# Deam0on/deepEMIA

Hardware: AMD Instinct MI355X
Metric: EM tiles/s (2048x2048, R101-FPN) (higher is better)
Workload: dtype f16x2

## Files before the change

deepemia_amd/_lib.py:

```python
from __future__ import annotations

import ctypes as C
import os
from pathlib import Path

_HERE = Path(__file__).resolve().parent
LIB_PATH = _HERE / "csrc" / ("libdeepemia_hip_dev.so" if os.environ.get("DEEPEMIA_DEV_LIB", "0") == "1" else "libdeepemia_hip.so")

F32, BF16, F32X3, BF16X2, F16X2, P32 = 0, 1, 2, 3, 4, 5
ACT_NONE, ACT_RELU, ACT_SIGMOID = 0, 1, 2
RES_NONE, RES_SAME, RES_UP2 = 0, 1, 2
MOP = {"fill": 1, "dilate": 2, "erode": 3, "drop_multi": 4, "flag_multi": 5, "gate": 6}


class HipExtensionMissing(RuntimeError):
    pass


class HipKernelError(RuntimeError):
    pass


class ConvDesc(C.Structure):
    _fields_ = [
# ... 8 lines not shown
    ]


class ConvP32Desc(C.Structure):
    _fields_ = [
        ("in_", C.c_void_p), ("in_meta", C.c_void_p), ("w", C.c_void_p), ("scale", C.c_void_p), ("bias", C.c_void_p),
        ("residual", C.c_void_p), ("res_meta", C.c_void_p), ("out", C.c_void_p), ("out_meta", C.c_void_p),
        ("wbound", C.c_float), ("bbound", C.c_float),
        ("N", C.c_int32), ("H", C.c_int32), ("W", C.c_int32), ("Cin", C.c_int32),
        ("Ho", C.c_int32), ("Wo", C.c_int32), ("Cout", C.c_int32), ("CoutPad", C.c_int32),
        ("KH", C.c_int32), ("KW", C.c_int32), ("stride", C.c_int32), ("pad", C.c_int32),
        ("act", C.c_int32), ("res_mode", C.c_int32), ("out_f32", C.c_int32), ("out_ld", C.c_int32), ("tile_hint", C.c_int32),
        ("head_w", C.c_void_p), ("head_b", C.c_void_p), ("head_out", C.c_void_p),
        ("head_n", C.c_int32), ("head_ld", C.c_int32), ("head_act", C.c_int32),
        ("groups", C.c_int32), ("group_rows", C.c_int32), ("row0", C.c_int32), ("single", C.c_int32),
    ]


class RpnDesc(C.Structure):
    _fields_ = [
        ("head", C.c_void_p * 5), ("H", C.c_int32 * 5), ("W", C.c_int32 * 5), ("stride", C.c_int32 * 5),
        ("cell_anchors", C.c_void_p), ("head_ld", C.c_int32), ("N", C.c_int32),
        ("img_h", C.c_int32), ("img_w", C.c_int32), ("pre_topk", C.c_int32), ("post_topk", C.c_int32),
        ("nms_thresh", C.c_float), ("out_boxes", C.c_void_p), ("out_scores", C.c_void_p),
        ("out_count", C.c_void_p), ("workspace", C.c_void_p),
    ]


class RoiAlignDesc(C.Structure):
    _fields_ = [
# ... 212 lines not shown
```

deepemia_amd/csrc/conv_p32.hip:

```cpp
#include <utility>
#include "common.h"
#ifndef P32_ABLATE
#define P32_ABLATE 0
#endif

#ifndef P32_HEAD_DIRECT
#define P32_HEAD_DIRECT 1
#endif
#ifndef P32_SINGLE
#define P32_SINGLE 0
#endif
#ifndef P32_DEV_TILES
#define P32_DEV_TILES 0
#endif
#ifndef P32_ST_AUX
#define P32_ST_AUX 0
#endif
#ifndef P32_RES_AUX
#define P32_RES_AUX 0
#endif
#ifndef P32_A_NT
#define P32_A_NT 0
#endif
#ifndef P32_FRAG_PIPE
// ... 11 lines not shown
    const void* res;
    const float* res_meta;
    void* out;
    float* out_meta;
    float wbound, bbound;
    int N, H, W, Cin, Ho, Wo, Cout, CoutPad, KH, KW, stride, pad;
    int act, res_mode, out_f32, out_ld;
    int M, HoWo, ntn, nwg, ksteps, taps;
    int kloop;
    unsigned in_bytes, w_bytes;
    unsigned out_bytes, res_bytes;
    const float* head_w;
    const float* head_b;
    float* head_out;
    int head_n, head_ld, head_act;
    int groups, group_rows, row0;
    int no_hk;
    int zero_low;
    int stagger_ticks;
    int resident;
};

typedef __attribute__((address_space(3))) void lds_void;

template <int OFF, int WAIT>
__device__ __forceinline__ void ds_read2_b128(f16x8& a, f16x8& b, unsigned addr_a, unsigned addr_b) {
    if constexpr (WAIT >= 0)
        asm volatile("ds_read_b128 %0, %2 offset:%4\n\tds_read_b128 %1, %3 offset:%4\n\ts_waitcnt lgkmcnt(%5)"
                     : "=&v"(a), "=&v"(b) : "v"(addr_a), "v"(addr_b), "n"(OFF), "n"(WAIT) : "memory");
    else
// ... 73 lines not shown
    if (p.res_mode != DEMIA_RES_NONE) { amax_res = p.res_meta[2 * gi]; s_res = p.res_meta[2 * gi + 1]; }
    post = uniform(1.0f / s_in);
    resi = uniform(p.res_mode != DEMIA_RES_NONE ? 1.0f / s_res : 0.f);
    sout = uniform(planes_out ? plane_scale(amax_in * p.wbound + p.bbound + amax_res) : 1.f);
}

__device__ __forceinline__ GroupScales load_group_scales(const ConvQ& p, int m0, bool planes_out) {
    GroupScales gs;
    gs.g0 = (m0 + p.row0) / p.group_rows;
    gs.b1 = (gs.g0 + 1) * p.group_rows - p.row0;
    gs.b2 = gs.b1 + p.group_rows;
    load_group_scale(p, gs.g0, planes_out, gs.post0, gs.resi0, gs.sout0);
    load_group_scale(p, gs.g0 + 1, planes_out, gs.post1, gs.resi1, gs.sout1);
    load_group_scale(p, gs.g0 + 2, planes_out, gs.post2, gs.resi2, gs.sout2);
    return gs;
}

template <int WM, int WN, int TM, int TN, bool HEAD, typename WriteRow>
__device__ __forceinline__ void p32_epilogue(const ConvQ& p, const GroupScales& gs, char* smem, WriteRow&& write_tile_row, int wm, int wn, int m0, int n0) {
    constexpr int BN = WN * TN * 32;
    const int tid = threadIdx.x, lane = tid & 63;
    constexpr int EROW = BN * 4 + 16;
    constexpr int GPR = BN / 8, RSTEP = 512 / GPR, ITEMS = WM * 32 / RSTEP;
    static_assert(512 % GPR == 0 && (WM * 32) % RSTEP == 0, "epilogue split");
    constexpr int BM_ = WM * TM * 32;
    static_assert(!HEAD || BN == 256, "the fused head needs a 256-wide tile");
    const bool planes_out = !HEAD && !p.out_f32;
    const int g0 = __builtin_amdgcn_readfirstlane(gs.g0), b1 = __builtin_amdgcn_readfirstlane(gs.b1), b2 = __builtin_amdgcn_readfirstlane(gs.b2);
    const float post0 = uniform(gs.post0), post1 = uniform(gs.post1), post2 = uniform(gs.post2);
    const float resi0 = uniform(gs.resi0), resi1 = uniform(gs.resi1), resi2 = uniform(gs.resi2);
// ... 64 lines not shown
#pragma unroll
        for (int k = 0; k < ITEMS; ++k) { ch[k] = rh[k]; cl[k] = rl[k]; }
        if (i + 1 < TM) load_res(i + 1);
        if (co < p.Cout) {
#pragma unroll
            for (int k = 0; k < ITEMS; ++k) {
                const int lr = r_first + k * RSTEP;
                const int m = row_of(i, k);
                if (m >= p.M) continue;
                const float4 x0 = *reinterpret_cast<const float4*>(smem + lr * EROW + g * 32);
                const float4 x1 = *reinterpret_cast<const float4*>(smem + lr * EROW + g * 32 + 16);
                float v[8] = {x0.x, x0.y, x0.z, x0.w, x1.x, x1.y, x1.z, x1.w};
                const int gd = (m >= b1) + (m >= b2);
                const float post = gd == 0 ? post0 : (gd == 1 ? post1 : post2);
#pragma unroll
                for (int q = 0; q < 8; ++q) v[q] = (v[q] * post) * sc[q] + bs[q];
                if (res_on) {
                    const float res_inv = gd == 0 ? resi0 : (gd == 1 ? resi1 : resi2);
#pragma unroll
                    for (int q = 0; q < 8; ++q) v[q] += ((float)ch[k][q] + (float)cl[k][q]) * res_inv;
                }
#pragma unroll
                for (int q = 0; q < 8; ++q) v[q] = fmaxf(v[q], act_lo);
                if (sigmoid_on) {
#pragma unroll
                    for (int q = 0; q < 8; ++q) v[q] = 1.0f / (1.0f + expf(-v[q]));
                }
                if (head_on) {
                    float acc_h[HMAX];
#pragma unroll
                    for (int j = 0; j < HMAX; ++j) {
// ... 145 lines not shown
        asm volatile("" ::: "memory");
        __builtin_amdgcn_wave_barrier();
        f16x8 ch[ITEMS], cl[ITEMS];
#pragma unroll
        for (int k = 0; k < ITEMS; ++k) {
            ch[k] = __builtin_bit_cast(f16x8, from_below(rh[k], rl[k]));
            cl[k] = __builtin_bit_cast(f16x8, from_above(rl[k], rh[k]));
        }
        if (i + 1 < TM) load_res(i + 1);
#pragma unroll
        for (int k = 0; k < ITEMS; ++k) {
            const int lr = r_first + k * RPI;
            const int m = row_of(i, k);
            const float4 x0 = *reinterpret_cast<const float4*>(wsm + lr * (LDW * 4) + (line * 4 + cj) * 32);
            const float4 x1 = *reinterpret_cast<const float4*>(wsm + lr * (LDW * 4) + (line * 4 + cj) * 32 + 16);
            typedef float f32x2 __attribute__((ext_vector_type(2)));
            f32x2 v2[4] = {{x0.x, x0.y}, {x0.z, x0.w}, {x1.x, x1.y}, {x1.z, x1.w}};
            const int gd = (m >= b1) + (m >= b2);
            const float post = gd == 0 ? post0 : (gd == 1 ? post1 : post2);
            const float res_inv = gd == 0 ? resi0 : (gd == 1 ? resi1 : resi2);
            const float s_out = gd == 0 ? sout0 : (gd == 1 ? sout1 : sout2);
            float v[8];
#pragma unroll
            for (int q = 0; q < 4; ++q) {
                const f32x2 scq = {sc[2 * q], sc[2 * q + 1]}, bsq = {bs[2 * q], bs[2 * q + 1]};
                const f32x2 t = (v2[q] * post) * scq + bsq;
                v[2 * q] = t.x;
                v[2 * q + 1] = t.y;
            }
#pragma unroll
            for (int q = 0; q < 8; ++q) {
                v[q] = fmaf((float)cl[k][q], res_inv, fmaf((float)ch[k][q], res_inv, v[q]));
                v[q] = fmaxf(v[q], act_lo);
            }
            if (sigmoid_on && !(P32_ABLATE & 256)) {
#pragma unroll
                for (int q = 0; q < 8; ++q) v[q] = 1.0f / (1.0f + expf(-v[q]));
            }
            f16x8 h, l;
            float vm = 0.f;
#pragma unroll
            for (int q = 0; q < 8; q += 2) {
                vm = fmaxf(vm, fmaxf(fabsf(v[q]), fabsf(v[q + 1])));
                const f32x2 y = f32x2{v[q], v[q + 1]} * s_out;
                h[q] = (_Float16)y.x;
                h[q + 1] = (_Float16)y.y;
                l[q] = (_Float16)fmaf(-(float)h[q], 1.0f, y.x);
                l[q + 1] = (_Float16)fmaf(-(float)h[q + 1], 1.0f, y.y);
            }
            if (single) l = f16x8{0, 0, 0, 0, 0, 0, 0, 0};
            vm = m < p.M ? vm : 0.f;
            vmax0 = fmaxf(vmax0, gd == 0 ? vm : 0.f);
            vmax1 = fmaxf(vmax1, gd == 1 ? vm : 0.f);
            vmax2 = fmaxf(vmax2, gd == 2 ? vm : 0.f);
            const u32x4 hu = __builtin_bit_cast(u32x4, h), lu = __builtin_bit_cast(u32x4, l);
            const u32x4 d0 = from_below(hu, lu);
            const u32x4 d1 = from_above(lu, hu);
            const unsigned off = (unsigned)(m - rs) * cbytes + lofs;
            if (P32_ABLATE & 64) {
                asm volatile("" :: "v"(d0), "v"(d1), "v"(off));
            } else {
                __builtin_amdgcn_raw_buffer_store_b128(d0, rs_out, off, 0, P32_ST_AUX);
                __builtin_amdgcn_raw_buffer_store_b128(d1, rs_out, off + cbytes, 0, P32_ST_AUX);
            }
// ... 66 lines not shown
    const int tile_n_ = n0 / BN;
    for (int o = tid; o < BM * HN; o += WM * WN * 64) {
        const int row = o / HN, j = o - row * HN;
        const int m = m0 + row;
        if (m >= p.M || j >= p.head_n) continue;
        float z = 0.f;
#pragma unroll
        for (int w = 0; w < WN; ++w) z += part[((long)w * BM + row) * HN + j];
        z += p.head_b[j];
        p.head_out[((long)m * p.ntn + tile_n_) * p.head_ld + j] =
            p.head_act == DEMIA_ACT_SIGMOID ? 1.0f / (1.0f + expf(-z)) : (p.head_act == DEMIA_ACT_RELU ? fmaxf(z, 0.f) : z);
    }
}


constexpr int EPI_GENERIC = 0, EPI_PLANES = 1, EPI_HEAD = 2;

template <int WM, int WN, int TM, int TN, bool M16 = true, int EPI = EPI_PLANES, int NST = 2, bool HK = false>
__global__ __launch_bounds__(WM * WN * 64, WM * WN == 8 ? 2 : 1) void conv_p32_kernel(const ConvQ p) {
    static_assert(NST == 2 || NST == 3, "two or three LDS stages");
    static_assert(!HK || (P32_SINGLE && M16 && NST == 2), "HK is a variant of the single-plane 16x16x32 kernel");
    static_assert(WM * WN == 8 || (WM * WN == 4 && EPI == EPI_PLANES), "eight waves, or four (planes epilogue only)");
    constexpr int NW = WM * WN;
    constexpr int BM = WM * TM * 32, BN = WN * TN * 32;
    constexpr int STAGE = (BM + BN) * 128;
    constexpr int NIA = BM / 8, NIB = BN / 8;

    extern __shared__ __attribute__((aligned(16))) char smem[];
    const int tid = threadIdx.x, lane = tid & 63;
    const int wave = __builtin_amdgcn_readfirstlane(tid >> 6);
    const int wm = wave / WN, wn = wave % WN;
// ... 324 lines not shown
            asm volatile("s_waitcnt lgkmcnt(0)\n\ts_barrier" ::: "memory");
        } else if (!BARRIER_IN_COMPUTE) {
            asm volatile("s_waitcnt vmcnt(0) lgkmcnt(0)\n\ts_barrier" ::: "memory");
        }
        st = NST == 2 ? (st ^ 1) : (st == 2 ? 0 : st + 1);
    }
#undef P32_ADVANCE

    if constexpr ((P32_ABLATE & 2048) != 0 && M16) {
#pragma unroll
        for (int i = 0; i < 2 * TM; ++i)
#pragma unroll
            for (int j = 0; j < 2 * TN; ++j) asm volatile("" :: "v"(acc16[i][j]));
        return;
    }
    if constexpr (EPI == EPI_PLANES) {
        if constexpr (M16) {
            p32_epilogue_planes<WM, WN, TM, TN>(p, gs, smem, [&](int i, float* e) { write_acc16<TN, TN * 32 + 4>(acc16[2 * i], acc16[2 * i + 1], e, lane); }, wm, wn, m0, n0);
        } else {
            p32_epilogue_planes<WM, WN, TM, TN>(p, gs, smem, [&](int i, float* e) { write_acc32<TN, TN * 32 + 4>(acc[i], e, lane); }, wm, wn, m0, n0);
        }
    } else if constexpr (M16 && HEAD && P32_HEAD_DIRECT) {
        if (p.act != DEMIA_ACT_SIGMOID && p.head_n <= 2)
            p32_epilogue_head_direct<WM, WN, TM, TN, 2>(p, gs, smem, acc16, wm, wn, m0, n0);
        else
            p32_epilogue<WM, WN, TM, TN, HEAD>(p, gs, smem, [&](int i, float* e) { write_acc16<TN, BN + 4>(acc16[2 * i], acc16[2 * i + 1], e, lane); }, wm, wn, m0, n0);
    } else if constexpr (M16) {
        p32_epilogue<WM, WN, TM, TN, HEAD>(p, gs, smem, [&](int i, float* e) { write_acc16<TN, BN + 4>(acc16[2 * i], acc16[2 * i + 1], e, lane); }, wm, wn, m0, n0);
    } else {
        p32_epilogue<WM, WN, TM, TN, HEAD>(p, gs, smem, [&](int i, float* e) { write_acc32<TN, BN + 4>(acc[i], e, lane); }, wm, wn, m0, n0);
    }
}

#if P32_DEV_TILES
#include "conv_p32_dev.inc"
#endif

template <int WM, int WN, int TM, int TN, bool M16 = true, int EPI = EPI_PLANES, int NST = 2, bool HK = false>
int launch_q_(ConvQ p, hipStream_t st) {
    constexpr int BM = WM * TM * 32, BN = WN * TN * 32;
    constexpr int stages = NST * (BM + BN) * 128, image = EPI == EPI_PLANES ? WM * WN * 32 * (TN * 128 + 16) : WM * 32 * (BN * 4 + 16);
    static_assert(stages <= 160 * 1024, "LDS");
    constexpr int smem = stages > image ? stages : image;
    p.ntn = p.CoutPad / BN;
    p.nwg = p.ntn * cdiv(p.M, BM);
    p.resident = 256 * (160 * 1024 / smem >= 2 ? 2 : 1);
    p.kloop = HK ? p.ksteps / 2 : p.ksteps;
    auto k = conv_p32_kernel<WM, WN, TM, TN, M16, EPI, NST, HK>;
    static bool attr_done = false;
    if (!attr_done) {
        (void)hipFuncSetAttribute(reinterpret_cast<const void*>(k), hipFuncAttributeMaxDynamicSharedMemorySize, smem);
        attr_done = true;
    }
    hipLaunchKernelGGL(k, dim3(p.nwg), dim3(WM * WN * 64), smem, st, p);
    DEMIA_CHECK_LAUNCH("conv_p32_kernel");
    return DEMIA_OK;
}
// ... 32 lines not shown
        const double t = predict_us(c, M, cout_pad, ksteps, residual);
        if (t < best_t) { best_t = t; best = c.id; }
    }
    return best;
}

}

#if P32_SINGLE
extern "C" int demia_conv2d_p32_single(const demia_conv_p32_desc* d, void* stream) {
#else
extern "C" int demia_conv2d_p32_single(const demia_conv_p32_desc* d, void* stream);
extern "C" int demia_conv2d_p32(const demia_conv_p32_desc* d, void* stream) {
    if (d && d->single) return demia_conv2d_p32_single(d, stream);
#endif
    DEMIA_REQUIRE(d && d->in && d->in_meta && d->w && (d->out || d->head_n > 0), "null pointer");
    DEMIA_REQUIRE(d->out_f32 || d->out_meta || d->head_n > 0, "P32 output needs out_meta");
    DEMIA_REQUIRE(d->Cin > 0 && d->Cin % 32 == 0, "Cin must be a multiple of 32");
    DEMIA_REQUIRE(d->CoutPad >= d->Cout && d->CoutPad % 64 == 0, "CoutPad must be a multiple of 64");
    DEMIA_REQUIRE(d->out_f32 || d->Cout % 32 == 0, "P32 output needs Cout % 32 == 0");
    DEMIA_REQUIRE(d->KH > 0 && d->KW > 0 && d->KH * d->KW <= 32 && d->stride > 0 && d->pad >= 0, "kernel geometry");
    DEMIA_REQUIRE(d->Ho == (d->H + 2 * d->pad - d->KH) / d->stride + 1, "Ho");
    DEMIA_REQUIRE(d->Wo == (d->W + 2 * d->pad - d->KW) / d->stride + 1, "Wo");
    DEMIA_REQUIRE(d->res_mode == DEMIA_RES_NONE || (d->residual && d->res_meta), "residual pointer");
    DEMIA_REQUIRE((long)d->N * d->Ho * d->Wo < (1L << 31), "M overflow");
    const long in_bytes = 128 + (long)d->N * d->H * d->W * d->Cin * 4;
    DEMIA_REQUIRE(in_bytes < (1L << 32), "input planes must stay below 4 GiB");
    const long w_bytes = (long)d->CoutPad * d->KH * d->KW * d->Cin * 4;
    DEMIA_REQUIRE(w_bytes < (1L << 31), "weight planes must stay below 2 GiB");
    ConvQ p;
    p.in = d->in; p.in_meta = d->in_meta; p.w = d->w; p.scale = d->scale; p.bias = d->bias;
    p.res = d->residual; p.res_meta = d->res_meta; p.out = d->out; p.out_meta = d->out_meta;
// ... 14 lines not shown
        static const char* env = getenv("DEMIA_P32_NO_HK");
        p.no_hk = (env && env[0] == '1') ? 1 : 0;
    }
    p.kloop = 0;
    p.resident = 256;
    p.groups = d->groups > 1 ? d->groups : 1;
    p.group_rows = p.groups > 1 ? d->group_rows : (1 << 29);
    p.row0 = p.groups > 1 ? d->row0 : 0;
    DEMIA_REQUIRE(p.groups == 1 || (d->group_rows >= 128 && d->row0 >= 0 && ((long)p.M + d->row0 + d->group_rows - 1) / d->group_rows <= p.groups),
                  "scale groups: group_rows >= 128 and the rows of this call must fall inside `groups` groups");
    p.head_w = d->head_w; p.head_b = d->head_b; p.head_out = d->head_out; p.head_n = d->head_n; p.head_ld = d->head_ld; p.head_act = d->head_act;
    if (d->head_n > 0) {
        DEMIA_REQUIRE(d->head_n <= 4 && d->head_w && d->head_b && d->head_out && d->head_ld >= d->head_n, "fused head: at most 4 rows, pointers, head_ld");
        DEMIA_REQUIRE(d->CoutPad % 256 == 0 && d->Cout == d->CoutPad && !d->out_f32, "fused head needs Cout % 256 == 0 and a planes layer");
    }
    p.stagger_ticks = 0;
#if P32_DEV_TILES
    {
        static const char* env = getenv("DEMIA_P32_STAGGER_US");
        p.stagger_ticks = env ? atoi(env) * 100 : 0;
    }
#endif
    if (p.M == 0) return DEMIA_OK;
    hipStream_t st = reinterpret_cast<hipStream_t>(stream);
    int tile = d->tile_hint ? d->tile_hint : choose_tile(p.M, d->CoutPad, p.ksteps, d->res_mode != DEMIA_RES_NONE, d->head_n > 0);
    const bool n256 = d->CoutPad % 256 == 0, n128 = d->CoutPad % 128 == 0;
    if (d->head_n > 0) {
        switch (tile) {
            case 1: return launch_q<2, 4, 4, 2, true, EPI_HEAD>(p, st);
            case 2: return launch_q<2, 4, 2, 2, true, EPI_HEAD>(p, st);
            default: return launch_q<1, 8, 6, 1, true, EPI_HEAD>(p, st);
        }
    }
    const int tile_bn = (tile == 9 || tile == 10 || tile == 11 || tile == 49) ? 64 : ((tile >= 6 && tile <= 8) || tile == 26 ? 128 : 256);
    const long out_bytes = 128 + (long)p.M * d->Cout * 4;
    long res_bytes = 0;
    if (d->res_mode == DEMIA_RES_SAME) res_bytes = out_bytes;
    if (d->res_mode == DEMIA_RES_UP2) res_bytes = 128 + (long)d->N * ((d->Ho + 1) / 2) * ((d->Wo + 1) / 2) * d->Cout * 4;
    const bool planes = !d->out_f32 && d->Cout % tile_bn == 0 && out_bytes < (1L << 32) - 512 && res_bytes < (1L << 32) - 512 &&
                        (long)(p.M + 256) * d->Cout * 4 + 256 < (1L << 32);
    p.out_bytes = (unsigned)out_bytes; p.res_bytes = (unsigned)res_bytes;
// ... 49 lines not shown
```

deepemia_amd/engine.py:

```python
from __future__ import annotations

import os

import ctypes as C
import math
from dataclasses import dataclass
from typing import Dict, List, Optional, Sequence, Tuple

import numpy as np
import torch

from . import _lib, p32
from ._lib import ACT_NONE, ACT_RELU, ACT_SIGMOID, BF16, BF16X2, F16X2, F32, F32X3, RES_NONE, RES_SAME, RES_UP2

RES_BLOCKS = {50: (3, 4, 6, 3), 101: (3, 4, 23, 3)}
PIXEL_MEAN = (103.530, 116.280, 123.675)
ANCHOR_SIZES = (32, 64, 128, 256, 512)
ANCHOR_RATIOS = (0.5, 1.0, 2.0)
STRIDES = (4, 8, 16, 32, 64)
DEFAULT_SINGLE_STAGES = ()
MASK_HEAD_STAGES = ("mask_fcn", "deconv")
STAGES = ("res2", "res3", "res4", "res5", "fpn_lateral", "fpn_output", "rpn_conv", "rpn_pred", "fc1", "fc2", "box_pred", "mask_fcn", "deconv")
BN_EPS = 1e-5
PRE_NMS_TOPK = 1000
# ... 213 lines not shown
        self._graphs: Dict[tuple, dict] = {}
        self._arena: Dict[tuple, list] = {}
        self._arena_key: Optional[tuple] = None
        self._arena_i = 0
        self._paste_static = None
        self.stem_mode = os.environ.get("DEEPEMIA_STEM", "fused") if self.p32 else "valu"
        self.stem_on_mfma = self.stem_mode in ("fused", "mfma")
        self.max_cached_shapes = max(1, int(os.environ.get("DEEPEMIA_MAX_CACHED_SHAPES", "3")))
        self._shape_lru: List[tuple] = []
        self.evictions = 0
        self.dt = BF16 if precision == "bf16" else F32
        self.tdt = torch.bfloat16 if precision == "bf16" else torch.float32
        self._tables: Dict[Tuple[int, int], dict] = {}
        self._cell = cell_anchor_table()
        self.roi_order = os.environ.get("DEEPEMIA_ROI_ORDER", "0") == "1"
        self.conv_events = None
        self.unmatched_keys: List[str] = []
        self._used = set()
        self._pack(state_dict)

    def _get(self, sd, key):
        if key not in sd:
            raise KeyError(f"checkpoint is missing '{key}' (expected Detectron2 0.6 Mask R-CNN R{self.depth}-FPN layout)")
        self._used.add(key)
        return sd[key].detach().to(torch.float32).cpu()

    def _conv(self, sd, prefix, stride=1, pad=0, norm=False, bias=False, weight=None, bias_t=None, stage: str = "") -> ConvLayer:
        w = self._get(sd, prefix + ".weight") if weight is None else weight
        cout, cin, kh, kw = w.shape
        cout_pad = (cout + 63) // 64 * 64 if self.p32 else (cout + 31) // 32 * 32
# ... 171 lines not shown
        m = self._meta_pool[self._meta_i]
        self._meta_i += 1
        return m

    def new_p32(self, shape, groups: Optional[int] = None) -> p32.P32:
        n = 1
        for d in shape:
            n *= int(d)
        buf = self._scratch(p32.HEADER_HALFS + 2 * n, torch.float16, zero_head=p32.HEADER_HALFS)
        return p32.P32(buf, self._meta_slot(self._groups if groups is None else groups), tuple(int(d) for d in shape))

    def dense(self, x) -> torch.Tensor:
        return p32.to_f32(x) if isinstance(x, p32.P32) else x.float()

    def conv_p32(self, x: p32.P32, L: ConvLayer, act=ACT_NONE, residual: Optional[p32.P32] = None, res_mode=RES_NONE,
                 out_f32: bool = False, out_ld: int = 0, tile_hint: int = 0, head=None):
        n, h, w, cin = x.shape
        assert cin == L.cin, (cin, L.cin)
        ho = (h + 2 * L.pad - L.kh) // L.stride + 1
        wo = (w + 2 * L.pad - L.kw) // L.stride + 1
        hw_ptr = hb_ptr = ho_ptr = hn = hld = hact = 0
        if head is not None:
            hw_t, hb_t, hld, hact = head
            hn = int(hw_t.shape[0])
            out = self._scratch(n * ho * wo * (L.cout // 256) * hld, torch.float32).view(n * ho * wo * (L.cout // 256), hld)
            hw_ptr, hb_ptr, ho_ptr = _lib.ptr(hw_t), _lib.ptr(hb_t), _lib.ptr(out)
            optr, ometa = 0, 0
        elif out_f32:
            ld = out_ld if out_ld > 0 else L.cout
            out = self._scratch(n * ho * wo * ld, torch.float32).view(n, ho, wo, ld)
            optr, ometa = _lib.ptr(out), 0
        else:
            out = self.new_p32((n, ho, wo, L.cout), x.groups)
            optr, ometa = _lib.ptr(out.buf), _lib.ptr(out.meta)
        pix_bytes = cin * 4
        limit = (1 << 32) - (1 << 20)
        chunks = [(0, n)]
# ... 4 lines not shown
            chunks = [(i, min(step, n - i)) for i in range(0, n, step)]
        ev = self.conv_events
        if ev is not None:
            e0, e1 = torch.cuda.Event(enable_timing=True), torch.cuda.Event(enable_timing=True)
            e0.record(torch.cuda.current_stream(self.device))
        groups = x.groups
        group_rows = (n * ho * wo) // groups
        assert groups == 1 or (group_rows * groups == n * ho * wo and (residual is None or residual.groups == groups)), (x.shape, groups)
        for c0, cn in chunks:
            d = _lib.ConvP32Desc(_lib.ptr(x.buf) + c0 * pix_bytes, _lib.ptr(x.meta), _lib.ptr(L.w3), _lib.ptr(L.scale3), _lib.ptr(L.bias),
                                 0 if residual is None else _lib.ptr(residual.buf) + c0 * L.cout * 4,
                                 0 if residual is None else _lib.ptr(residual.meta),
                                 (optr + c0 * (ld if out_f32 else L.cout) * 4) if optr else 0, ometa, L.wbound, L.bbound, cn, h, w, cin,
                                 ho, wo, L.cout, L.cout_pad, L.kh, L.kw, L.stride, L.pad, act, res_mode, 1 if out_f32 else 0, out_ld,
                                 tile_hint, hw_ptr, hb_ptr, (ho_ptr + c0 * (L.cout // 256) * hld * 4) if ho_ptr else 0, hn, hld, hact,
                                 groups, group_rows, c0, L.single)
            _lib.check(self.lib.demia_conv2d_p32(C.byref(d), self._stream()), "demia_conv2d_p32")
        if ev is not None:
            e1.record(torch.cuda.current_stream(self.device))
            nbytes = (n * h * w * cin * 4 + L.cout_pad * L.kh * L.kw * cin * 4 + n * ho * wo * L.cout * 4 +
                      (0 if residual is None else residual.pixels * residual.channels * 4))
            ev.append((e0, e1, 2.0 * n * ho * wo * L.cout * L.kh * L.kw * cin, "f16" if L.single else self.precision, nbytes))
        return out

    def conv(self, x, L: ConvLayer, act=ACT_NONE, residual=None, res_mode=RES_NONE,
             out_dtype=None, out: Optional[torch.Tensor] = None, out_ld: int = 0, tile_hint: int = 0):
        if self.p32:
            return self.conv_p32(x, L, act, residual, res_mode, out_f32=out_dtype is not None, out_ld=out_ld, tile_hint=tile_hint)
        n, h, w, cin = x.shape
        assert cin == L.cin, (cin, L.cin)
        ho = (h + 2 * L.pad - L.kh) // L.stride + 1
        wo = (w + 2 * L.pad - L.kw) // L.stride + 1
        odt = self.tdt if out_dtype is None else out_dtype
        ld = out_ld if out_ld > 0 else L.cout
        if out is None:
            out = torch.empty((n, ho, wo, ld), dtype=odt, device=self.device)
        use3 = L.w3 is not None and odt == torch.float32
# ... 144 lines not shown
        h5, w5 = p5.shape[1], p5.shape[2]
        if self.p32:
            p6 = self.new_p32((b, (h5 - 1) // 2 + 1, (w5 - 1) // 2 + 1, 256))
            p6 = p32.P32(p6.buf, p5.meta, p6.shape)
            _lib.check(self.lib.demia_subsample2(_lib.ptr(p5.buf) + 128, _lib.ptr(p6.buf) + 128, b, h5, w5, 256, F32, st), "demia_subsample2")
            feats["p6"] = p6
            return feats
        p6 = torch.empty((b, (h5 - 1) // 2 + 1, (w5 - 1) // 2 + 1, 256), dtype=self.tdt, device=self.device)
        _lib.check(self.lib.demia_subsample2(_lib.ptr(p5), _lib.ptr(p6), b, h5, w5, 256, self.dt, st), "demia_subsample2")
        feats["p6"] = p6
        return feats

    def rpn(self, feats, newh: int, neww: int):
        b = feats["p2"].shape[0]
        heads = []
        for name in ("p2", "p3", "p4", "p5", "p6"):
            t = self.conv(feats[name], self.rpn_conv, act=ACT_RELU)
            heads.append(self.conv(t, self.rpn_pred, out_dtype=torch.float32, out_ld=16))
        boxes = torch.empty((b, POST_NMS_TOPK, 4), dtype=torch.float32, device=self.device)
        scores = torch.empty((b, POST_NMS_TOPK), dtype=torch.float32, device=self.device)
        count = torch.empty((b,), dtype=torch.int32, device=self.device)
        ws = torch.empty((int(self.lib.demia_rpn_workspace_bytes(b)),), dtype=torch.uint8, device=self.device)
        d = _lib.RpnDesc()
        for i, hd in enumerate(heads):
            d.head[i] = _lib.ptr(hd)
            d.H[i], d.W[i], d.stride[i] = hd.shape[1], hd.shape[2], STRIDES[i]
        d.cell_anchors = self._cell.ctypes.data
        d.head_ld, d.N, d.img_h, d.img_w = 16, b, newh, neww
        d.pre_topk, d.post_topk, d.nms_thresh = PRE_NMS_TOPK, POST_NMS_TOPK, RPN_NMS_THRESH
        d.out_boxes, d.out_scores, d.out_count, d.workspace = _lib.ptr(boxes), _lib.ptr(scores), _lib.ptr(count), _lib.ptr(ws)
        _lib.check(self.lib.demia_rpn_proposals(C.byref(d), self._stream()), "demia_rpn_proposals")
# ... 175 lines not shown
```

include/deepemia_hip.h:

```cpp
#ifndef DEEPEMIA_HIP_H
#define DEEPEMIA_HIP_H

#include <stdint.h>

#ifdef __cplusplus
extern "C" {
#endif

#define DEMIA_OK 0
#define DEMIA_EINVAL (-1)
#define DEMIA_ELAUNCH (-2)

#define DEMIA_F32 0
#define DEMIA_BF16 1
#define DEMIA_F32X3 2
#define DEMIA_BF16X2 3
#define DEMIA_F16X2 4
#define DEMIA_P32 5

#define DEMIA_ACT_NONE 0
#define DEMIA_ACT_RELU 1
#define DEMIA_ACT_SIGMOID 2

#define DEMIA_RES_NONE 0
// ... 41 lines not shown
    float* out_meta;
    float wbound, bbound;
    int32_t N, H, W, Cin;
    int32_t Ho, Wo, Cout, CoutPad;
    int32_t KH, KW, stride, pad;
    int32_t act, res_mode;
    int32_t out_f32;
    int32_t out_ld;
    int32_t tile_hint;
    const float* head_w;
    const float* head_b;
    float* head_out;
    int32_t head_n, head_ld, head_act;
    int32_t groups, group_rows, row0;
    int32_t single;
} demia_conv_p32_desc;
int demia_conv2d_p32(const demia_conv_p32_desc* d, void* stream);

int demia_resize_h_u8(const uint8_t* src, uint8_t* tmp, int N, int H, int W, int newW,
                      const int32_t* xmin, const int32_t* xsize, const int32_t* xk, int ksx, void* stream);
int demia_resize_v_norm(const uint8_t* tmp, void* dst, int N, int H, int newW, int newH, int PH, int PW,
                        const int32_t* ymin, const int32_t* ysize, const int32_t* yk, int ksy,
                        const float* mean3, int dtype, void* stream);

int demia_resize_linear_u8(const uint8_t* src, uint8_t* dst, int N, int H, int W, int out_h, int out_w,
                           const int32_t* xofs, const int16_t* ialpha, const int32_t* yofs, const int16_t* ibeta,
                           void* stream);

int demia_stem_conv(const void* in, const void* w, const float* scale, const float* bias, void* mid,
                    int N, int PH, int PW, int dtype, void* stream);
// ... 222 lines not shown
```

Measured before the change: 719.5.

## Fuse RPN 1x1 prediction conv into the 3x3 RPN conv epilogue

Adds an epilogue mode to the P32 conv kernel that, for the 256-channel RPN 3x3 conv, writes the activated tile as f16 hi/lo planes into LDS and immediately runs the following 1x1 prediction layer (up to 16 outputs) with MFMA, storing f32 head outputs directly. The goal is to avoid materialising the 256-channel intermediate in HBM and to save a second kernel launch per FPN level. The fused path is on by default for f16x2 and adds LDS pressure, an extra barrier per row tile, and a new tile choice. The shared elementwise code is factored into a helper.

```diff
diff --git a/deepemia_amd/_lib.py b/deepemia_amd/_lib.py
--- a/deepemia_amd/_lib.py
+++ b/deepemia_amd/_lib.py
@@ -46,6 +46,7 @@
         ("head_w", C.c_void_p), ("head_b", C.c_void_p), ("head_out", C.c_void_p),
         ("head_n", C.c_int32), ("head_ld", C.c_int32), ("head_act", C.c_int32),
         ("groups", C.c_int32), ("group_rows", C.c_int32), ("row0", C.c_int32), ("single", C.c_int32),
+        ("head_planes", C.c_void_p), ("head_scale", C.c_void_p), ("head_bias", C.c_void_p), ("head_cout", C.c_int32),
     ]
 
 
diff --git a/deepemia_amd/csrc/conv_p32.hip b/deepemia_amd/csrc/conv_p32.hip
--- a/deepemia_amd/csrc/conv_p32.hip
+++ b/deepemia_amd/csrc/conv_p32.hip
@@ -49,6 +49,10 @@
     const float* head_b;
     float* head_out;
     int head_n, head_ld, head_act;
+    const void* hp_w;
+    const float* hp_scale;
+    const float* hp_bias;
+    int hp_cout;
     int groups, group_rows, row0;
     int no_hk;
     int zero_low;
@@ -152,6 +156,41 @@
     load_group_scale(p, gs.g0 + 1, planes_out, gs.post1, gs.resi1, gs.sout1);
     load_group_scale(p, gs.g0 + 2, planes_out, gs.post2, gs.resi2, gs.sout2);
     return gs;
+}
+
+__device__ __forceinline__ float scale_shift(float acc, float post, float sc, float bs) { return (acc * post) * sc + bs; }
+__device__ __forceinline__ void planes_item(const float4 x0, const float4 x1, float post, float res_inv, float s_out, const float (&sc)[8],
+                                            const float (&bs)[8], const f16x8 ch, const f16x8 cl, float act_lo, bool sigmoid_on,
+                                            f16x8& h, f16x8& l, float& vm) {
+    typedef float f32x2 __attribute__((ext_vector_type(2)));
+    f32x2 v2[4] = {{x0.x, x0.y}, {x0.z, x0.w}, {x1.x, x1.y}, {x1.z, x1.w}};
+    float v[8];
+#pragma unroll
+    for (int q = 0; q < 4; ++q) {
+        const f32x2 scq = {sc[2 * q], sc[2 * q + 1]}, bsq = {bs[2 * q], bs[2 * q + 1]};
+        const f32x2 t = (v2[q] * post) * scq + bsq;
+        v[2 * q] = t.x;
+        v[2 * q + 1] = t.y;
+    }
+#pragma unroll
+    for (int q = 0; q < 8; ++q) {
+        v[q] = fmaf((float)cl[q], res_inv, fmaf((float)ch[q], res_inv, v[q]));
+        v[q] = fmaxf(v[q], act_lo);
+    }
+    if (sigmoid_on && !(P32_ABLATE & 256)) {
+#pragma unroll
+        for (int q = 0; q < 8; ++q) v[q] = 1.0f / (1.0f + expf(-v[q]));
+    }
+    vm = 0.f;
+#pragma unroll
+    for (int q = 0; q < 8; q += 2) {
+        vm = fmaxf(vm, fmaxf(fabsf(v[q]), fabsf(v[q + 1])));
+        const f32x2 y = f32x2{v[q], v[q + 1]} * s_out;
+        h[q] = (_Float16)y.x;
+        h[q + 1] = (_Float16)y.y;
+        l[q] = (_Float16)fmaf(-(float)h[q], 1.0f, y.x);
+        l[q + 1] = (_Float16)fmaf(-(float)h[q + 1], 1.0f, y.y);
+    }
 }
 
 template <int WM, int WN, int TM, int TN, bool HEAD, typename WriteRow>
@@ -246,7 +285,7 @@
                 const int gd = (m >= b1) + (m >= b2);
                 const float post = gd == 0 ? post0 : (gd == 1 ? post1 : post2);
 #pragma unroll
-                for (int q = 0; q < 8; ++q) v[q] = (v[q] * post) * sc[q] + bs[q];
+                for (int q = 0; q < 8; ++q) v[q] = scale_shift(v[q], post, sc[q], bs[q]);
                 if (res_on) {
                     const float res_inv = gd == 0 ? resi0 : (gd == 1 ? resi1 : resi2);
 #pragma unroll
@@ -422,40 +461,13 @@
             const int m = row_of(i, k);
             const float4 x0 = *reinterpret_cast<const float4*>(wsm + lr * (LDW * 4) + (line * 4 + cj) * 32);
             const float4 x1 = *reinterpret_cast<const float4*>(wsm + lr * (LDW * 4) + (line * 4 + cj) * 32 + 16);
-            typedef float f32x2 __attribute__((ext_vector_type(2)));
-            f32x2 v2[4] = {{x0.x, x0.y}, {x0.z, x0.w}, {x1.x, x1.y}, {x1.z, x1.w}};
             const int gd = (m >= b1) + (m >= b2);
             const float post = gd == 0 ? post0 : (gd == 1 ? post1 : post2);
             const float res_inv = gd == 0 ? resi0 : (gd == 1 ? resi1 : resi2);
             const float s_out = gd == 0 ? sout0 : (gd == 1 ? sout1 : sout2);
-            float v[8];
-#pragma unroll
-            for (int q = 0; q < 4; ++q) {
-                const f32x2 scq = {sc[2 * q], sc[2 * q + 1]}, bsq = {bs[2 * q], bs[2 * q + 1]};
-                const f32x2 t = (v2[q] * post) * scq + bsq;
-                v[2 * q] = t.x;
-                v[2 * q + 1] = t.y;
-            }
-#pragma unroll
-            for (int q = 0; q < 8; ++q) {
-                v[q] = fmaf((float)cl[k][q], res_inv, fmaf((float)ch[k][q], res_inv, v[q]));
-                v[q] = fmaxf(v[q], act_lo);
-            }
-            if (sigmoid_on && !(P32_ABLATE & 256)) {
-#pragma unroll
-                for (int q = 0; q < 8; ++q) v[q] = 1.0f / (1.0f + expf(-v[q]));
-            }
             f16x8 h, l;
-            float vm = 0.f;
-#pragma unroll
-            for (int q = 0; q < 8; q += 2) {
-                vm = fmaxf(vm, fmaxf(fabsf(v[q]), fabsf(v[q + 1])));
-                const f32x2 y = f32x2{v[q], v[q + 1]} * s_out;
-                h[q] = (_Float16)y.x;
-                h[q + 1] = (_Float16)y.y;
-                l[q] = (_Float16)fmaf(-(float)h[q], 1.0f, y.x);
-                l[q + 1] = (_Float16)fmaf(-(float)h[q + 1], 1.0f, y.y);
-            }
+            float vm;
+            planes_item(x0, x1, post, res_inv, s_out, sc, bs, ch[k], cl[k], act_lo, sigmoid_on, h, l, vm);
             if (single) l = f16x8{0, 0, 0, 0, 0, 0, 0, 0};
             vm = m < p.M ? vm : 0.f;
             vmax0 = fmaxf(vmax0, gd == 0 ? vm : 0.f);
@@ -552,7 +564,115 @@
 }
 
 
-constexpr int EPI_GENERIC = 0, EPI_PLANES = 1, EPI_HEAD = 2;
+template <int WM, int WN, int TM, int TN>
+struct HeadPlanesLds {
+    static constexpr int LDW = TN * 32 + 4, ROWS = WM * 32;
+    static constexpr int STG = WM * WN * 32 * LDW * 4, IMG = ROWS * 8 * 128, WB = 8 * 16 * 128;
+    static constexpr int BYTES = STG + IMG + WB;
+};
+template <int WM, int WN, int TM, int TN, typename WriteRow>
+__device__ __forceinline__ void p32_epilogue_head_planes(const ConvQ& p, const GroupScales& gs, char* smem, WriteRow&& write_tile_row, int wm, int wn, int m0) {
+    typedef HeadPlanesLds<WM, WN, TM, TN> L;
+    static_assert(WN * TN == 8 && WM * WN == 8, "one N tile of 256 channels, eight waves");
+    constexpr int LDW = L::LDW, ROWS = L::ROWS;
+    constexpr int PPW = 8 / TN, RPI = 2 * PPW, ITEMS = 32 / RPI;
+    const int tid = threadIdx.x, lane = tid & 63;
+    const int wave = __builtin_amdgcn_readfirstlane(tid >> 6);
+    char* const wsm = smem + wave * (32 * LDW * 4);
+    char* const img = smem + L::STG;
+    char* const wimg = img + L::IMG;
+    const int b1 = __builtin_amdgcn_readfirstlane(gs.b1), b2 = __builtin_amdgcn_readfirstlane(gs.b2);
+    const float post0 = uniform(gs.post0), post1 = uniform(gs.post1), post2 = uniform(gs.post2);
+    const float sout0 = uniform(gs.sout0), sout1 = uniform(gs.sout1), sout2 = uniform(gs.sout2);
+    const float ipost0 = uniform(1.0f / sout0), ipost1 = uniform(1.0f / sout1), ipost2 = uniform(1.0f / sout2);
+    u32x4 wreg[2];
+#pragma unroll
+    for (int q = 0; q < 2; ++q) {
+        const int c = tid + q * 512, g = c >> 7, row = (c >> 3) & 15, ck = c & 7;
+        wreg[q] = *reinterpret_cast<const u32x4*>(reinterpret_cast<const char*>(p.hp_w) + g * 8192 + row * 128 + ck * 16);
+    }
+    const int cj = lane & 3, rs = (lane >> 2) & 1, lg = lane >> 3;
+    const int line = lg % TN;
+    const int r_first = (lg / TN) * 2 + rs;
+    const int cgrp = wn * TN + line;
+    const int co = (cgrp * 4 + cj) * 8;
+    float sc[8], bs[8];
+#pragma unroll
+    for (int q = 0; q < 8; ++q) {
+        sc[q] = p.scale ? p.scale[co + q] : 1.0f;
+        bs[q] = p.bias ? p.bias[co + q] : 0.0f;
+    }
+    const bool sigmoid_on = p.act == DEMIA_ACT_SIGMOID;
+    const float act_lo = p.act == DEMIA_ACT_RELU ? 0.f : -INFINITY;
+    const f16x8 zero8 = {0, 0, 0, 0, 0, 0, 0, 0};
+    const int r16 = lane & 15, kq = lane >> 4, fsw = (r16 >> 1) & 7;
+    const bool c_ok = r16 < p.hp_cout;
+    const float hsc = (p.hp_scale && c_ok) ? p.hp_scale[r16] : 1.0f;
+    const float hbs = (p.hp_bias && c_ok) ? p.hp_bias[r16] : 0.0f;
+#pragma unroll
+    for (int i = 0; i < TM; ++i) {
+        asm volatile("" ::: "memory");
+        __builtin_amdgcn_wave_barrier();
+        write_tile_row(i, reinterpret_cast<float*>(wsm));
+        asm volatile("" ::: "memory");
+        __builtin_amdgcn_wave_barrier();
+        f16x8 h[ITEMS], l[ITEMS];
+#pragma unroll
+        for (int k = 0; k < ITEMS; ++k) {
+            const int lr = r_first + k * RPI;
+            const int m = m0 + wm * (TM * 32) + i * 32 + lr;
+            const float4 x0 = *reinterpret_cast<const float4*>(wsm + lr * (LDW * 4) + (line * 4 + cj) * 32);
+            const float4 x1 = *reinterpret_cast<const float4*>(wsm + lr * (LDW * 4) + (line * 4 + cj) * 32 + 16);
+            const int gd = (m >= b1) + (m >= b2);
+            const float post = gd == 0 ? post0 : (gd == 1 ? post1 : post2);
+            const float s_out = gd == 0 ? sout0 : (gd == 1 ? sout1 : sout2);
+            float vm;
+            planes_item(x0, x1, post, 0.f, s_out, sc, bs, zero8, zero8, act_lo, sigmoid_on, h[k], l[k], vm);
+        }
+        if (i > 0) __syncthreads();
+#pragma unroll
+        for (int k = 0; k < ITEMS; ++k) {
+            const int R = wm * 32 + r_first + k * RPI, sw = (R >> 1) & 7;
+            char* ln = img + (cgrp * ROWS + R) * 128;
+            *reinterpret_cast<f16x8*>(ln + ((cj ^ sw) * 16)) = h[k];
+            *reinterpret_cast<f16x8*>(ln + (((4 + cj) ^ sw) * 16)) = l[k];
+        }
+        if (i == 0) {
+#pragma unroll
+            for (int q = 0; q < 2; ++q) {
+                const int c = tid + q * 512, g = c >> 7, row = (c >> 3) & 15, ck = c & 7;
+                *reinterpret_cast<u32x4*>(wimg + g * 2048 + row * 128 + ((ck ^ ((row >> 1) & 7)) * 16)) = wreg[q];
+            }
+        }
+        __syncthreads();
+        if (wave < ROWS / 16) {
+            f32x4 c = {0.f, 0.f, 0.f, 0.f};
+#pragma unroll
+            for (int g = 0; g < 8; ++g) {
+                const char* ab = img + (g * ROWS + wave * 16 + r16) * 128;
+                const char* bb = wimg + g * 2048 + r16 * 128;
+                const f16x8 ah = *reinterpret_cast<const f16x8*>(ab + ((kq ^ fsw) * 16));
+                const f16x8 al = *reinterpret_cast<const f16x8*>(ab + (((4 + kq) ^ fsw) * 16));
+                const f16x8 bh = *reinterpret_cast<const f16x8*>(bb + ((kq ^ fsw) * 16));
+                const f16x8 bl = *reinterpret_cast<const f16x8*>(bb + (((4 + kq) ^ fsw) * 16));
+                c = __builtin_amdgcn_mfma_f32_16x16x32_f16(ah, bl, c, 0, 0, 0);
+                c = __builtin_amdgcn_mfma_f32_16x16x32_f16(al, bh, c, 0, 0, 0);
+                c = __builtin_amdgcn_mfma_f32_16x16x32_f16(ah, bh, c, 0, 0, 0);
+            }
+#pragma unroll
+            for (int r = 0; r < 4; ++r) {
+                const int R = wave * 16 + kq * 4 + r;
+                const int m = m0 + (R >> 5) * (TM * 32) + i * 32 + (R & 31);
+                const int gd = (m >= b1) + (m >= b2);
+                const float ipost = gd == 0 ? ipost0 : (gd == 1 ? ipost1 : ipost2);
+                const float z = fmaxf(scale_shift(c[r], ipost, hsc, hbs), -INFINITY);
+                if (m < p.M && c_ok) p.head_out[(long)m * p.head_ld + r16] = z;
+            }
+        }
+    }
+}
+
+constexpr int EPI_GENERIC = 0, EPI_PLANES = 1, EPI_HEAD = 2, EPI_HEAD_PLANES = 3;
 
 template <int WM, int WN, int TM, int TN, bool M16 = true, int EPI = EPI_PLANES, int NST = 2, bool HK = false>
 __global__ __launch_bounds__(WM * WN * 64, WM * WN == 8 ? 2 : 1) void conv_p32_kernel(const ConvQ p) {
@@ -907,7 +1027,10 @@
             for (int j = 0; j < 2 * TN; ++j) asm volatile("" :: "v"(acc16[i][j]));
         return;
     }
-    if constexpr (EPI == EPI_PLANES) {
+    if constexpr (EPI == EPI_HEAD_PLANES) {
+        static_assert(M16, "the fused 1x1 layer rides on the 16x16x32 kernel");
+        p32_epilogue_head_planes<WM, WN, TM, TN>(p, gs, smem, [&](int i, float* e) { write_acc16<TN, TN * 32 + 4>(acc16[2 * i], acc16[2 * i + 1], e, lane); }, wm, wn, m0);
+    } else if constexpr (EPI == EPI_PLANES) {
         if constexpr (M16) {
             p32_epilogue_planes<WM, WN, TM, TN>(p, gs, smem, [&](int i, float* e) { write_acc16<TN, TN * 32 + 4>(acc16[2 * i], acc16[2 * i + 1], e, lane); }, wm, wn, m0, n0);
         } else {
@@ -932,8 +1055,9 @@
 template <int WM, int WN, int TM, int TN, bool M16 = true, int EPI = EPI_PLANES, int NST = 2, bool HK = false>
 int launch_q_(ConvQ p, hipStream_t st) {
     constexpr int BM = WM * TM * 32, BN = WN * TN * 32;
-    constexpr int stages = NST * (BM + BN) * 128, image = EPI == EPI_PLANES ? WM * WN * 32 * (TN * 128 + 16) : WM * 32 * (BN * 4 + 16);
-    static_assert(stages <= 160 * 1024, "LDS");
+    constexpr int stages = NST * (BM + BN) * 128, image = EPI == EPI_HEAD_PLANES ? HeadPlanesLds<WM, WN, TM, TN>::BYTES
+                                                         : (EPI == EPI_PLANES ? WM * WN * 32 * (TN * 128 + 16) : WM * 32 * (BN * 4 + 16));
+    static_assert(stages <= 160 * 1024 && image <= 160 * 1024, "LDS");
     constexpr int smem = stages > image ? stages : image;
     p.ntn = p.CoutPad / BN;
     p.nwg = p.ntn * cdiv(p.M, BM);
@@ -996,8 +1120,8 @@
 extern "C" int demia_conv2d_p32(const demia_conv_p32_desc* d, void* stream) {
     if (d && d->single) return demia_conv2d_p32_single(d, stream);
 #endif
-    DEMIA_REQUIRE(d && d->in && d->in_meta && d->w && (d->out || d->head_n > 0), "null pointer");
-    DEMIA_REQUIRE(d->out_f32 || d->out_meta || d->head_n > 0, "P32 output needs out_meta");
+    DEMIA_REQUIRE(d && d->in && d->in_meta && d->w && (d->out || d->head_n > 0 || d->head_planes), "null pointer");
+    DEMIA_REQUIRE(d->out_f32 || d->out_meta || d->head_n > 0 || d->head_planes, "P32 output needs out_meta");
     DEMIA_REQUIRE(d->Cin > 0 && d->Cin % 32 == 0, "Cin must be a multiple of 32");
     DEMIA_REQUIRE(d->CoutPad >= d->Cout && d->CoutPad % 64 == 0, "CoutPad must be a multiple of 64");
     DEMIA_REQUIRE(d->out_f32 || d->Cout % 32 == 0, "P32 output needs Cout % 32 == 0");
@@ -1042,6 +1166,16 @@
         DEMIA_REQUIRE(d->head_n <= 4 && d->head_w && d->head_b && d->head_out && d->head_ld >= d->head_n, "fused head: at most 4 rows, pointers, head_ld");
         DEMIA_REQUIRE(d->CoutPad % 256 == 0 && d->Cout == d->CoutPad && !d->out_f32, "fused head needs Cout % 256 == 0 and a planes layer");
     }
+    p.hp_w = d->head_planes; p.hp_scale = d->head_scale; p.hp_bias = d->head_bias; p.hp_cout = d->head_cout;
+    if (d->head_planes) {
+#if P32_SINGLE
+        DEMIA_REQUIRE(false, "fused 1x1 layer (head_planes): not in the single-plane build");
+#endif
+        DEMIA_REQUIRE(d->head_n == 0 && d->head_out && d->head_cout >= 1 && d->head_cout <= 16 && d->head_ld >= d->head_cout,
+                      "fused 1x1 layer: head_n == 0, head_out, 1 <= head_cout <= 16, head_ld >= head_cout");
+        DEMIA_REQUIRE(d->Cout == 256 && d->CoutPad == 256 && !d->out_f32 && d->res_mode == DEMIA_RES_NONE,
+                      "fused 1x1 layer needs a planes layer of exactly 256 channels without residual");
+    }
     p.stagger_ticks = 0;
 #if P32_DEV_TILES
     {
@@ -1051,8 +1185,19 @@
 #endif
     if (p.M == 0) return DEMIA_OK;
     hipStream_t st = reinterpret_cast<hipStream_t>(stream);
-    int tile = d->tile_hint ? d->tile_hint : choose_tile(p.M, d->CoutPad, p.ksteps, d->res_mode != DEMIA_RES_NONE, d->head_n > 0);
+    int tile = d->tile_hint ? d->tile_hint : choose_tile(p.M, d->CoutPad, p.ksteps, d->res_mode != DEMIA_RES_NONE, d->head_n > 0 || d->head_planes);
     const bool n256 = d->CoutPad % 256 == 0, n128 = d->CoutPad % 128 == 0;
+#if !P32_SINGLE
+    if (d->head_planes) {
+        if (!d->tile_hint && cdiv(p.M, 128) <= 128) tile = 15;
+        switch (tile) {
+            case 1: return launch_q<2, 4, 4, 2, true, EPI_HEAD_PLANES>(p, st);
+            case 2: return launch_q<2, 4, 2, 2, true, EPI_HEAD_PLANES>(p, st);
+            case 15: return launch_q<1, 8, 2, 1, true, EPI_HEAD_PLANES>(p, st);
+            default: return launch_q<1, 8, 6, 1, true, EPI_HEAD_PLANES>(p, st);
+        }
+    }
+#endif
     if (d->head_n > 0) {
         switch (tile) {
             case 1: return launch_q<2, 4, 4, 2, true, EPI_HEAD>(p, st);
diff --git a/deepemia_amd/engine.py b/deepemia_amd/engine.py
--- a/deepemia_amd/engine.py
+++ b/deepemia_amd/engine.py
@@ -251,6 +251,7 @@
         self._tables: Dict[Tuple[int, int], dict] = {}
         self._cell = cell_anchor_table()
         self.roi_order = os.environ.get("DEEPEMIA_ROI_ORDER", "0") == "1"
+        self.rpn_fused = os.environ.get("DEEPEMIA_RPN_FUSED", "1") != "0"
         self.conv_events = None
         self.unmatched_keys: List[str] = []
         self._used = set()
@@ -452,13 +453,22 @@
         return p32.to_f32(x) if isinstance(x, p32.P32) else x.float()
 
     def conv_p32(self, x: p32.P32, L: ConvLayer, act=ACT_NONE, residual: Optional[p32.P32] = None, res_mode=RES_NONE,
-                 out_f32: bool = False, out_ld: int = 0, tile_hint: int = 0, head=None):
+                 out_f32: bool = False, out_ld: int = 0, tile_hint: int = 0, head=None, then: Optional[ConvLayer] = None):
         n, h, w, cin = x.shape
         assert cin == L.cin, (cin, L.cin)
         ho = (h + 2 * L.pad - L.kh) // L.stride + 1
         wo = (w + 2 * L.pad - L.kw) // L.stride + 1
         hw_ptr = hb_ptr = ho_ptr = hn = hld = hact = 0
-        if head is not None:
+        tp_ptr = ts_ptr = tb_ptr = tcout = 0
+        if then is not None:
+            assert head is None and residual is None and not out_f32, "a fused 1x1 layer follows a plain planes layer"
+            assert L.cout == L.cout_pad == 256 == then.cin and then.cout <= 16 and not L.single and not then.single, (L.cout, then.cout)
+            assert (then.kh, then.kw, then.stride, then.pad) == (1, 1, 1, 0), "the fused consumer is a 1x1 stride-1 layer"
+            hld = out_ld if out_ld > 0 else then.cout
+            out = self._scratch(n * ho * wo * hld, torch.float32).view(n, ho, wo, hld)
+            ho_ptr, tp_ptr, ts_ptr, tb_ptr, tcout = _lib.ptr(out), _lib.ptr(then.w3), _lib.ptr(then.scale3), _lib.ptr(then.bias), then.cout
+            optr, ometa, out_ld = 0, 0, 0
+        elif head is not None:
             hw_t, hb_t, hld, hact = head
             hn = int(hw_t.shape[0])
             out = self._scratch(n * ho * wo * (L.cout // 256) * hld, torch.float32).view(n * ho * wo * (L.cout // 256), hld)
@@ -493,13 +503,17 @@
                                  (optr + c0 * (ld if out_f32 else L.cout) * 4) if optr else 0, ometa, L.wbound, L.bbound, cn, h, w, cin,
                                  ho, wo, L.cout, L.cout_pad, L.kh, L.kw, L.stride, L.pad, act, res_mode, 1 if out_f32 else 0, out_ld,
                                  tile_hint, hw_ptr, hb_ptr, (ho_ptr + c0 * (L.cout // 256) * hld * 4) if ho_ptr else 0, hn, hld, hact,
-                                 groups, group_rows, c0, L.single)
+                                 groups, group_rows, c0, L.single, tp_ptr, ts_ptr, tb_ptr, tcout)
             _lib.check(self.lib.demia_conv2d_p32(C.byref(d), self._stream()), "demia_conv2d_p32")
         if ev is not None:
             e1.record(torch.cuda.current_stream(self.device))
             nbytes = (n * h * w * cin * 4 + L.cout_pad * L.kh * L.kw * cin * 4 + n * ho * wo * L.cout * 4 +
                       (0 if residual is None else residual.pixels * residual.channels * 4))
-            ev.append((e0, e1, 2.0 * n * ho * wo * L.cout * L.kh * L.kw * cin, "f16" if L.single else self.precision, nbytes))
+            flops = 2.0 * n * ho * wo * L.cout * L.kh * L.kw * cin
+            if then is not None:
+                nbytes += then.cout_pad * then.cin * 4 + n * ho * wo * (then.cout - L.cout) * 4
+                flops += 2.0 * n * ho * wo * then.cout * then.cin
+            ev.append((e0, e1, flops, "f16" if L.single else self.precision, nbytes))
         return out
 
     def conv(self, x, L: ConvLayer, act=ACT_NONE, residual=None, res_mode=RES_NONE,
@@ -674,7 +688,11 @@
     def rpn(self, feats, newh: int, neww: int):
         b = feats["p2"].shape[0]
         heads = []
+        fused = self.rpn_fused and self.precision == "f16x2" and not self.rpn_conv.single and not self.rpn_pred.single
         for name in ("p2", "p3", "p4", "p5", "p6"):
+            if fused:
+                heads.append(self.conv_p32(feats[name], self.rpn_conv, act=ACT_RELU, then=self.rpn_pred, out_ld=16))
+                continue
             t = self.conv(feats[name], self.rpn_conv, act=ACT_RELU)
             heads.append(self.conv(t, self.rpn_pred, out_dtype=torch.float32, out_ld=16))
         boxes = torch.empty((b, POST_NMS_TOPK, 4), dtype=torch.float32, device=self.device)
diff --git a/include/deepemia_hip.h b/include/deepemia_hip.h
--- a/include/deepemia_hip.h
+++ b/include/deepemia_hip.h
@@ -79,6 +79,10 @@
     int32_t head_n, head_ld, head_act;
     int32_t groups, group_rows, row0;
     int32_t single;
+    const void* head_planes;
+    const float* head_scale;
+    const float* head_bias;
+    int32_t head_cout;
 } demia_conv_p32_desc;
 int demia_conv2d_p32(const demia_conv_p32_desc* d, void* stream);
 
```

After: 726.8, median of 6. 1.01x the previous value.
